# indygreg/python-zstandard

Measured on AMD Instinct MI355X. Metric: GB/s uncompressed throughput, batch decompress of 128 KiB level-3 frames (the decompress half of BASELINE.json's metric; the compress half on the same inputs is this line's 'compress' object), higher is better.
Workload: dtype u8

## Files before the change

### python-zstandard_amd/csrc/zhip_decode_pipeline.hpp

```cpp
#pragma once
#include "zhip_decode_kernel.hpp"

ZH_DEV void zp_pack_fse(ZdLDS& L, uint32_t* T, uint32_t llLog, uint32_t ofLog, uint32_t mlLog)
{
    const uint32_t lane = zh_lane();
    for (uint32_t u = lane; u < ZP_FSE_CELLS / 2; u += 64) {
        const uint32_t lg = u < 256 ? llLog : u < 512 ? mlLog : ofLog;
        const uint32_t local = (2 * u) & (u < 512 ? 511u : 255u);
        uint32_t pair = 0;
        for (uint32_t k = 0; k < 2; k++) {
            uint32_t cell = 0;
            if (local + k < (1u << lg)) {
                const uint32_t e = L.fse[2 * u + k];
                cell = ((e >> 19) << 10) | (((e & 1023) + (1u << lg)) >> ((e >> 10) & 15));
            }
            pair |= cell << (16 * k);
        }
        T[u] = pair;
    }
}

struct ZpHdr { uint32_t pos, blockMax, hasChecksum, skippable; uint64_t fcs; };
ZH_DEV int zp_frame_header(const ZhipPipeArgs& a, const uint8_t* src, uint32_t srcSize, ZpHdr& h)
{
// ... 867 lines not shown
#ifndef ZQ_FRAMES
#define ZQ_FRAMES 15
#endif
#define ZQ_ROWS 32
struct ZpSeqQLDS { uint32_t ring[(ZQ_ROWS + 1) * 16]; uint32_t llInfo[36]; uint32_t mlInfo[53]; uint32_t spare; uint8_t tab[ZQ_FRAMES * ZP_K2_STRIDE]; };

ZH_DEV uint32_t zq_field(const uint32_t* col, int32_t q, uint32_t width)
{
    const uint32_t* w = (const uint32_t*)((const uint8_t*)col + (zh_bfe((uint32_t)q, 5, 5) << 6));
    return zh_bfe(zh_alignbit(w[16], w[0], (uint32_t)q), 0, width);
}
ZH_DEV void zq_commit(uint32_t* col, int32_t off, const ZpVec16& v)
{
    const uint32_t r0 = ((uint32_t)off >> 2) & (ZQ_ROWS - 1);
    uint32_t* q = col + (r0 << 4);
    q[0] = v.a; q[16] = v.b; q[32] = v.c; q[48] = v.d;
    if (r0 == 0) col[ZQ_ROWS << 4] = v.a;
}
ZH_DEV ZpVec16 zq_fetch(const uint8_t* p0, int32_t off) { return *(const ZpVec16*)(p0 + (uint32_t)(off < 0 ? 0 : off)); }

#ifndef ZQ_FENCES
#define ZQ_FENCES 1
#endif
#if ZQ_FENCES >= 1
#define ZQ_F1() ZH_SCHED_FENCE()
#else
#define ZQ_F1() do { } while (0)
#endif
#if ZQ_FENCES >= 2
#define ZQ_F2() ZH_SCHED_FENCE()
#else
#define ZQ_F2() do { } while (0)
#endif
template <bool MB>
ZH_DEVFN void zp_seqq_body(const ZhipPipeArgs& a, ZpSeqQLDS& L)
{
    const uint32_t lane = zh_lane(), role = lane & 3, slot = lane >> 2;
    if (lane < 36) L.llInfo[lane] = zc_llBase[lane] | ((uint32_t)zc_llBits[lane] << 24);
    if (lane < 53) L.mlInfo[lane] = zc_mlBase[lane] | ((uint32_t)zc_mlBits[lane] << 24);
    if (lane == 0) L.spare = 512;
    zh_sync();
    const bool isOF = role == 0, isSpare = role == 3;
    const uint32_t* const info = role == 1 ? L.mlInfo : L.llInfo;
    const uint32_t tabOff = role == 0 ? ZP_FSE_OF : role == 1 ? ZP_FSE_ML : ZP_FSE_LL;
    const uint32_t total = a.counters[1];
    const uint32_t nGroups = (total + ZQ_FRAMES - 1) / ZQ_FRAMES;
    for (;;) {
        const uint32_t g = zh_first(zh_atomic_add(a.counters + 3, lane == 0 ? 1u : 0u));
        if (g >= nGroups) break;
        const uint32_t k = g * ZQ_FRAMES + slot;
        const bool active = slot < ZQ_FRAMES && k < total;
        const uint32_t i = active ? a.order[k] : 0xFFFFFFFFu;
        const uint32_t logs0 = active ? a.meta[i].logs : 0u;
        zh_sync();
        for (uint32_t j = 0; j < ZQ_FRAMES; j++) {
            const uint32_t fj = zh_shfl(i, 4 * j);
            if (fj == 0xFFFFFFFFu) break;
            const bool sharedT = (zh_shfl(logs0, 4 * j) & ZP_LOGS_SHARED) != 0;
            const uint32_t* src = sharedT ? (const uint32_t*)a.dictTables->fseK2 : (const uint32_t*)(a.fseTables + (size_t)fj * ZP_FSE_CELLS);
            uint32_t* dstw = (uint32_t*)(L.tab + (size_t)j * ZP_K2_STRIDE);
            uint32_t r[ZP_FSE_CELLS / 128];
#pragma unroll
            for (uint32_t q = 0; q < ZP_FSE_CELLS / 128; q++) r[q] = src[lane + 64 * q];
#pragma unroll
            for (uint32_t q = 0; q < ZP_FSE_CELLS / 128; q++) dstw[lane + 64 * q] = r[q];
        }
        uint32_t* const col = L.ring + (active ? slot : 0u);
        const bool idle = isSpare || !active;
        const uint16_t* const Tm = idle ? (const uint16_t*)&L.spare : (const uint16_t*)(L.tab + (size_t)slot * ZP_K2_STRIDE) + tabOff;
        ZdMeta* const m = a.meta + (active ? i : 0u);
        const uint32_t fi = active ? (MB ? a.itemFrame[i] : i) : 0u;
        const uint32_t f = a.first + fi;
        uint32_t nbSeq = 0, logs = 0;
        int32_t pos = 0, pb = -(1 << 30), fin = 0;
        const uint8_t* p0 = nullptr;
        bool ok = active;
        ZpVec16 v0, v1; v0.a = v0.b = v0.c = v0.d = 0; v1 = v0;
// ... 3 lines not shown
            const uint8_t* p = src + m->seqOff; const uint8_t* end = src + m->seqEnd;
            const uint32_t size = (uint32_t)(end - p);
            logs = m->logs;
            const uint32_t lastB = size ? p[size - 1] : 0u;
            if (lastB == 0) ok = false;
            else {
                nbSeq = m->nbSeq;
                const uint32_t mis = (uint32_t)((uintptr_t)p & 15);
                p0 = p - mis; fin = (int32_t)(8 * mis);
                const int32_t topByte = (int32_t)(mis + size) - 1;
                tb = topByte & ~15;
                v0 = zq_fetch(p0, tb - 16 * (int32_t)role); v1 = zq_fetch(p0, tb - 16 * (int32_t)(role + 4));
                pb = tb - 128;
                pos = 8 * topByte + zh_highbit32(lastB);
            }
        }
        if (ok) { zq_commit(col, tb - 16 * (int32_t)role, v0); zq_commit(col, tb - 16 * (int32_t)(role + 4), v1); }
        zh_sync();
        const uint32_t llLog = logs & 255, ofLog = (logs >> 8) & 255, mlLog = (logs >> 16) & 255;
        const uint32_t myLog = idle ? 9u : role == 0 ? ofLog : role == 1 ? mlLog : llLog;
        const uint32_t kk = 31 - myLog, size = 1u << myLog;
        const uint16_t* const Tb = Tm - size;
        uint32_t state;
        {   const uint32_t initOff = role == 0 ? llLog : role == 1 ? llLog + ofLog : 0u;
            state = idle ? size : size + zq_field(col, pos - (int32_t)(initOff + myLog), myLog);
            pos -= (int32_t)(llLog + ofLog + mlLog); }
        const uint32_t nTrips = zh_first(zh_wave_max(nbSeq)) + 5;
        uint32_t rep0 = 1, rep1 = 4, rep2 = 8;
        if (a.dictEntropy) { rep0 = a.dictEntropy->rep[0]; rep1 = a.dictEntropy->rep[1]; rep2 = a.dictEntropy->rep[2]; }
        if (MB && active && a.frameRecs[fi].firstItem != i) { rep0 = ZP_SYM_REP(0); rep1 = ZP_SYM_REP(1); rep2 = ZP_SYM_REP(2); }
        uint32_t fin0 = rep0, fin1 = rep1, fin2 = rep2;
        rep0 = zh_opaque(rep0); rep1 = zh_opaque(rep1); rep2 = zh_opaque(rep2);
        ZpVec16* outp;
        {
            const uint32_t per = ((nTrips - 5 + 3) & ~3u) + 8;
            const uint32_t nAct = (uint32_t)zh_popc64(zh_ballot(active)) >> 2;
            const uint32_t need16 = per * nAct / 2;
            const uint32_t room16 = zh_first(zh_atomic_add(a.counters + 7, lane == 0 ? need16 : 0u));
            const uint32_t room = room16 * 2;
            if ((uint64_t)room16 + need16 + a.counters[8] > a.arenaBudget16) {
                if (active && isOF) { m->path = 2; if (!MB) { const uint32_t q = zh_atomic_add(a.fallbackCount, 1u); a.fallbackList[q] = f; } }
                zh_sync();
                continue;
            }
            const uint32_t start = room + slot * per + 4;
            if (active && isOF) a.bases[2 * (size_t)i] = start;
            outp = (ZpVec16*)(a.seqArena + (isOF && active ? (size_t)start - 4 : (size_t)room + per - 4));
        }
        const uint32_t outStep = isOF && active ? 2u : 0u;
        uint32_t g1lo = 0, g1hi = 0, g2lo = 0, g2hi = 0, g3lo = 0, g3hi = 0;
        ZpVec16 w0, w1; w0.a = w0.b = w0.c = w0.d = 0; w1 = w0;
        int32_t boff = ZP_NOBLK, posEnd = pos; ZpVec16 blk = v0;
        uint32_t pe0 = 0, pe1 = 0, pqE = 0, pbits = 0, pbase = 1;
        for (uint32_t n0 = 0; n0 < nTrips; n0 += 4) {
            zh_sync();
            if (boff != ZP_NOBLK) { zq_commit(col, boff, blk); boff = ZP_NOBLK; }
            {
                const int32_t t = pb + 128 - (((pos >> 5) << 2) + 4);
                if ((int32_t)(role * 16) <= t) { boff = pb - 16 * (int32_t)role; blk = zq_fetch(p0, boff); }
                int32_t cnt = (t >> 4) + 1; cnt = cnt < 0 ? 0 : cnt > 4 ? 4 : cnt;
                pb -= 16 * cnt; }
#pragma unroll
            for (uint32_t u = 0; u < 4; u++) {
                const uint32_t n = n0 + u;
                const uint32_t cell = Tb[state];
                ZQ_F1();
                const uint32_t val = pbase + zh_bfe(zh_alignbit(pe1, pe0, pqE), 0, pbits);
                const uint32_t mlv = zh_quad<1>(val), llv = zh_quad<2>(val);
                const uint32_t idx = val - 1 + (llv == 0);
                const uint32_t vm3 = val - 3;
                const uint32_t newOff = vm3 < ZP_OF_LIMIT ? vm3 : ZP_OF_LIMIT;
                const uint32_t c3 = val > 3 ? newOff : rep0 - 1;
                uint32_t offset = idx == 2 ? rep2 : c3; offset = idx == 1 ? rep1 : offset; offset = idx == 0 ? rep0 : offset;
                ZQ_F2();
                const uint32_t sym = cell >> 10, x = cell & 1023;
                const uint32_t inf = info[sym];
                const uint32_t nb = (uint32_t)__builtin_clz(x) - kk;
                ZQ_F2();
                rep2 = idx <= 1 ? rep2 : rep1; rep1 = idx == 0 ? rep1 : rep0; rep0 = offset;
                if (MB) {
                    const bool wasLast = n == nbSeq;
                    fin0 = wasLast ? rep0 : fin0; fin1 = wasLast ? rep1 : fin1; fin2 = wasLast ? rep2 : fin2;
                }
                {   const uint32_t plo = llv | (mlv << 17), phi = (mlv >> 15) | (offset << 3);
                    if (u == 0) {
                        w0.a = g1lo; w0.b = g1hi; w0.c = g2lo; w0.d = g2hi; w1.a = g3lo; w1.b = g3hi; w1.c = plo; w1.d = phi;
#if defined(ZQ_DIAG_NOSTORE)
                        outp += outStep;
#elif defined(ZQ_NT_STORE)
                        {   typedef uint32_t zq_v4 __attribute__((ext_vector_type(4)));
                            zq_v4 t0 = { w0.a, w0.b, w0.c, w0.d }, t1 = { w1.a, w1.b, w1.c, w1.d };
                            __builtin_nontemporal_store(t0, (zq_v4*)outp); __builtin_nontemporal_store(t1, (zq_v4*)(outp + 1)); outp += outStep; }
#else
                        outp[0] = w0; outp[1] = w1; outp += outStep;
#endif
                    } else if (u == 1) { g1lo = plo; g1hi = phi; } else if (u == 2) { g2lo = plo; g2hi = phi; } else { g3lo = plo; g3hi = phi; } }
                ZQ_F2();
                const uint32_t bits = isOF ? sym : inf >> 24;
                const uint32_t P = zh_quad_add<0xCF>(zh_quad_add<0xD3>(bits, bits), bits);
                const uint32_t R = zh_quad_add<0xFE>(zh_quad_add<0xF9>(nb, nb), nb);
                const uint32_t totE = zh_quad<2>(P), totN = zh_quad<0>(R);
                const int32_t pE = pos - (int32_t)totE;
                const int32_t qS = pE - (int32_t)R, qE = pos - (int32_t)P;
                const uint32_t* const wS = (const uint32_t*)((const uint8_t*)col + (zh_bfe((uint32_t)qS, 5, 5) << 6));
                const uint32_t* const wE = (const uint32_t*)((const uint8_t*)col + (zh_bfe((uint32_t)qE, 5, 5) << 6));
                const uint32_t s0 = wS[0], s1 = wS[16];
                pe0 = wE[0]; pe1 = wE[16];
                ZQ_F2();
                pqE = (uint32_t)qE; pbits = bits;
                posEnd = n + 1 == nbSeq ? pE : posEnd;
                pos = pE - (int32_t)totN;
                pbase = isOF ? 1u << (sym & 31) : inf & 0xFFFFFFu;
                ZQ_F2();
                state = (x << nb) + zh_bfe(zh_alignbit(s1, s0, (uint32_t)qS), 0, nb);
            }
            ZH_KEEP4(w0.a, w0.b, w0.c, w0.d); ZH_KEEP4(w1.a, w1.b, w1.c, w1.d);
        }
        if (active && isOF) {
            const int err = !ok ? ZE_CORRUPTION : posEnd != fin ? ZE_CORRUPTION : 0;
            if (err) { m->status = err; m->path = 0; if (!MB) { a.status[f] = err; a.outSizes[f] = 0; } }
            if (MB) { uint32_t* r = a.itemReps + 4 * (size_t)i; r[0] = fin0; r[1] = fin1; r[2] = fin2; }
        }
        zh_sync();
    }
}

#ifndef ZP_ASM_BYTES
#define ZP_ASM_BYTES ZD_ASM_BYTES
#endif
struct ZpExecLDS {
    uint8_t asmb[ZP_ASM_BYTES + 64]; uint16_t mBeg[64]; uint16_t mEnd[64]; uint32_t misc[8];
#if defined(ZP_K3_DIAG_FLOOR) && defined(ZP_FLOOR_LDSPAD)
    uint8_t floorPad[ZP_FLOOR_LDSPAD];
#endif
    uint16_t uEnd[64], uLit[64], dstL[64], dstM[64], lenL[64], lenM[64]; uint32_t srcL[64], srcM[64];
};

ZH_DEV void zp_ld32_lds(const uint8_t* q, uint32_t len, uint64_t r[4])
{
    r[0] = zh_ld64(q); r[1] = zh_ld64(q + 8); r[2] = zh_ld64(q + 16);
    r[3] = zh_ld64(q + (len >= 8 ? len - 8 : 0u));
}

#ifndef ZP_LIT_SHORT
#define ZP_LIT_SHORT 16
#endif
#ifndef ZP_FAR_SHORT
#define ZP_FAR_SHORT 16
#endif
#ifndef ZP_K3_NT
#define ZP_K3_NT 0
#endif
#if ZP_K3_NT & 1
#define ZP_SEQ_LD(p) zh_ldq_nt(p)
#define ZP_LIT_LD64(p) zh_ld64_nt(p)
#else
#define ZP_SEQ_LD(p) (*(p))
#define ZP_LIT_LD64(p) zh_ld64(p)
#endif
#if ZP_K3_NT & 2
#define ZP_FAR_LD64(p) zh_ld64_nt(p)
#else
#define ZP_FAR_LD64(p) zh_ld64(p)
#endif
#define ZD_TP(P, i) do { if (PROF) ZD_T(P, i); } while (0)
ZH_DEV uint32_t zp_sym_resolve(uint32_t v, uint32_t R0, uint32_t R1, uint32_t R2)
{
    if (v <= ZP_OF_LIMIT) return v;
    if (v > ZP_SYM_TOP) return 0xFFFFFFFFu;
    const uint32_t k = (v - (ZP_OF_LIMIT + 1)) >> 23;
    const uint32_t d = ZP_SYM_REP(k) - v;
    const uint32_t r = k == 0 ? R0 : k == 1 ? R1 : R2;
    return r > d ? r - d : 0xFFFFFFFFu;
}

#define ZP_BSYNC() zh_sync()
#ifndef ZP_HIST_KEEP
#define ZP_HIST_KEEP ((ZP_ASM_BYTES * 5u / 16u) & ~15u)
#define ZP_HIST_SLIDE (2u * ZP_HIST_KEEP + 16u)
#endif
static_assert((ZP_HIST_SLIDE >= 2 * ZP_HIST_KEEP + 16 || ZP_HIST_KEEP == 0) && ZP_HIST_KEEP % 16 == 0 && ZP_HIST_SLIDE < ZP_ASM_BYTES, "the slide's source and destination must not overlap");
template <bool DICT, bool PROF, bool MB>
ZH_DEVFN int zp_exec_block(const ZhipPipeArgs& a, ZpExecLDS& L, const ZdMeta& m, uint32_t t, const uint8_t* src, uint8_t* dst, uint32_t cap, uint64_t cap64,
                           uint32_t blockMax, uint32_t& opRef, uint32_t R0, uint32_t R1, uint32_t R2, ZdProf& P)
{
    const uint32_t lane = zh_lane();
    const uint64_t* seqs = a.seqArena + a.bases[2 * (size_t)t];
    const bool litRLE = m.litMode == 2;
    const uint32_t rleByte = m.litOff;
    const uint8_t* litPtr = m.litMode == 0 ? src + m.litOff : a.litArena + (size_t)a.bases[2 * (size_t)t + 1] * 16;
    const uint8_t* const dictEnd = DICT ? a.dictContent + a.dictContentSize : dst;
    const uint32_t dictSize = DICT ? a.dictContentSize : 0u;
    uint32_t hOff = 0;
    uint8_t* asmb = L.asmb;
    const uint32_t blockStart = MB ? opRef : 0u;
    uint32_t op = blockStart, lp = 0, done = 0;
    uint32_t carry = 0;
    const uint32_t nbSeq = m.nbSeq;
    uint64_t qNext = lane < nbSeq ? ZP_SEQ_LD(seqs + lane) : 0;
    const uint32_t lane0 = lane;
    while (done < nbSeq) {
        const uint32_t avail = nbSeq - done < 64 ? nbSeq - done : 64;
        uint32_t myLL = 0, myML = 0, myOF = 1;
        if (lane < avail) { const uint64_t q = qNext; myLL = ZP_SEQ_LL(q); myML = ZP_SEQ_ML(q); myOF = ZP_SEQ_OF(q); if (MB) myOF = zp_sym_resolve(myOF, R0, R1, R2); }
        if (MB && zh_ballot(lane < avail && myOF == ZP_OF_LIMIT)) return ZP_RC_FALLBACK;
        uint32_t incL = zh_scan_add(myLL), incT = zh_scan_add(myLL + myML);
        const uint64_t fits = zh_ballot(lane < avail && incT + carry <= ZP_ASM_BYTES - hOff);
        uint32_t cnt = (uint32_t)zh_popc64(fits);
        const bool big = cnt == 0;
        if (big) cnt = 1;
        qNext = done + cnt + lane < nbSeq ? ZP_SEQ_LD(seqs + done + cnt + lane) : 0;
        const bool act = lane < cnt;
        if (!act) { myLL = 0; myML = 0; myOF = 1; }
        const uint32_t totL = zh_bcast(incL, cnt - 1), totT = zh_bcast(incT, cnt - 1);
        if (lp + totL > m.litSize) return ZE_CORRUPTION;
        if ((uint64_t)op + totT > cap) return ZE_DST_TOO_SMALL;
        if (op + totT - blockStart > blockMax) return ZE_CORRUPTION;
        const uint32_t litStart = lp + incL - myLL;
        const uint32_t ob = op - carry;
        const uint32_t oRel = incT - (myLL + myML) + carry, mRel = oRel + myLL;
        if (zh_ballot(act && myOF - 1 >= ob + mRel + dictSize)) return ZE_CORRUPTION;
        if (big) {
            if (lane < carry) dst[ob + lane] = asmb[lane];
            carry = 0;
            zd_fence();
            const uint32_t bll = zh_bcast(myLL, 0), bml = zh_bcast(myML, 0), bof = zh_bcast(myOF, 0);
            if (litRLE) zd_fill_wave(dst + op, rleByte, bll); else zd_copy_wave(dst + op, litPtr + lp, bll);
            zd_fence();
            zd_match_wave(dst, dictEnd, op + bll, bof, bml);
            zd_fence();
            op += totT; lp += totL; done += 1;
            hOff = 0; asmb = L.asmb;
            continue;
        }
        ZD_TP(P, ZP_STAGE);
        const int32_t sAbs = (int32_t)(ob + mRel) - (int32_t)myOF;
        const bool hasM = act && myML > 0;
        const bool farM = hasM && sAbs + (int32_t)myML <= (int32_t)ob;
        uint32_t nearSkip = 0;
        {
            uint64_t rl[4], rm[4];
            const bool shortL = act && myLL > 0 && myLL <= ZP_LIT_SHORT;
            const bool arenaLit = m.litMode != 0;
            if (arenaLit && !litRLE) {
// ... 99 lines not shown
                            if (c == span) span += span;
                        }
                    }
                    pending = false;
                }
                uint64_t newDone = zh_ballot(ready);
                for (uint64_t lm = longReady; lm; lm &= lm - 1) {
                    const uint32_t pf = (uint32_t)zh_ctz64(lm);
                    const uint32_t Frel = zh_shfl(mRel, pf), fml = zh_shfl(myML, pf), fof = zh_shfl(myOF, pf);
                    const int32_t fs = (int32_t)(ob + Frel) - (int32_t)fof;
                    if (fof >= 64) {
                        for (uint32_t c = 0; c < fml; c += 64) {
                            const uint32_t j = c + lane;
                            if (j < fml) { const int32_t sp = fs + (int32_t)j; asmb[Frel + j] = sp >= (int32_t)(ob - hOff) ? asmb[sp - (int32_t)ob] : (DICT ? (uint8_t)zd_hist_byte(dst, dictEnd, sp) : dst[sp]); }
                            if (fof < fml) ZP_BSYNC();
                        }
                    } else {
                        uint32_t idx = lane % fof; const uint32_t adv = 64 % fof;
                        for (uint32_t j = lane; j < fml; j += 64) {
                            const int32_t sp = fs + (int32_t)idx;
                            asmb[Frel + j] = sp >= (int32_t)(ob - hOff) ? asmb[sp - (int32_t)ob] : (DICT ? (uint8_t)zd_hist_byte(dst, dictEnd, sp) : dst[sp]);
                            idx += adv; if (idx >= fof) idx -= fof;
                        }
                    }
                    if (lane == pf) pending = false;
                    newDone |= 1ull << pf;
                    if (lm & (lm - 1)) ZP_BSYNC();
                }
                doneMask |= newDone;
            }
            ZP_BSYNC();
        }
        ZD_TP(P, ZP_EXEC2);
        qNext = zh_opaque64(qNext);
        const uint32_t totB = totT + carry, whole = totB & ~15u;
        {
            uint8_t* out = dst + ob;
            const uint32_t j0 = lane * 16;
            if (j0 < whole) { const zh_v16 v = *(const zh_v16*)(asmb + j0); *(zh_v16*)(out + j0) = v; }
            if (whole > 1024) for (uint32_t j = j0 + 1024; j < whole; j += 1024) { const zh_v16 v = *(const zh_v16*)(asmb + zh_opaque(j)); *(zh_v16*)(out + j) = v; }
        }
        carry = totB - whole;
        hOff += whole;
        ZP_BSYNC();
        if (hOff > ZP_HIST_SLIDE) {
            const uint32_t s0 = hOff - ZP_HIST_KEEP, n = ZP_HIST_KEEP + carry;
            for (uint32_t j = lane * 16; j < n; j += 1024) { const zh_v16 v = *(const zh_v16*)(L.asmb + s0 + j); *(zh_v16*)(L.asmb + j) = v; }
            hOff = ZP_HIST_KEEP;
            ZP_BSYNC();
        }
        asmb = L.asmb + hOff;
        ZD_TP(P, ZP_FLUSH);
        op += totT; lp += totL; done += cnt;
    }
    if (lane < carry) dst[op - carry + lane] = asmb[lane];
    zd_fence();
    const uint32_t rest = m.litSize - lp;
    if ((uint64_t)op + rest > cap) return ZE_DST_TOO_SMALL;
    if (op + rest - blockStart > blockMax) return ZE_CORRUPTION;
    if (litRLE) zd_fill_wave(dst + op, rleByte, rest); else zd_copy_wave(dst + op, litPtr + lp, rest);
    op += rest;
    opRef = op;
    return 0;
}


ZH_DEVFN int zp_exec_frame_end(ZpExecLDS& L, const uint8_t* dst, uint32_t op, uint32_t fcsLo, uint32_t fcsHi, uint32_t hasChecksum, uint32_t checksum, uint32_t ckLater)
{
    const uint32_t lane = zh_lane();
    const uint64_t fcs = (uint64_t)fcsLo | ((uint64_t)fcsHi << 32);
    if (fcs != ~0ull && fcs != op) return ZE_CORRUPTION;
    if ((hasChecksum & 1) && !ckLater) {
        zd_fence();
        zh_sync();
        if (zh_opaque(lane) == 0) L.misc[0] = (uint32_t)ze_xxh64(dst, op);
        zh_sync();
        const uint32_t digest = zh_first(L.misc[0]);
        zh_sync();
        if (digest != checksum) return ZE_CHECKSUM_WRONG;
    }
    return 0;
}

#ifdef ZP_K3_DIAG_FLOOR
#include "../../tests/ubench/k3_floor_diag.hpp"
#endif
template <bool DICT, bool PROF>
ZH_DEVFN int zp_exec_frame(const ZhipPipeArgs& a, ZpExecLDS& L, uint32_t i, uint32_t* pProduced, ZdProf& P)
{
    const ZdMeta m = a.meta[i];
    const uint32_t f = a.first + i;
    const uint8_t* src = a.src + a.srcSegs[2 * (size_t)f];
    uint8_t* dst = a.dst + a.dstSegs[2 * (size_t)f];
    const uint64_t cap64 = a.dstSegs[2 * (size_t)f + 1];
    const uint32_t cap = cap64 > 0x7FFFFFFFull ? 0x7FFFFFFFu : (uint32_t)cap64;
    uint32_t op = 0;
#ifdef ZP_K3_DIAG_FLOOR
// ... 100 lines not shown
```

### python-zstandard_amd/csrc/zhip_format.hpp

```cpp
#pragma once
#include <stdint.h>

enum {
    ZE_OK = 0, ZE_GENERIC = 1, ZE_PREFIX_UNKNOWN = 10, ZE_FRAMEPARAM_UNSUPPORTED = 14, ZE_WINDOW_TOO_LARGE = 16,
    ZE_CORRUPTION = 20, ZE_CHECKSUM_WRONG = 22, ZE_LITERALS_HEADER_WRONG = 24, ZE_DICT_CORRUPTED = 30,
    ZE_DICT_WRONG = 32, ZE_PARAM_UNSUPPORTED = 40, ZE_PARAM_OUTOFBOUND = 42, ZE_TABLELOG_TOO_LARGE = 44, ZE_MAXSYMBOL_TOO_LARGE = 46,
    ZE_MAXSYMBOL_TOO_SMALL = 48, ZE_MEMORY = 64, ZE_DST_TOO_SMALL = 70, ZE_SRC_SIZE_WRONG = 72
};

#define ZF_MAGIC 0xFD2FB528u
#define ZF_MAGIC_SKIPPABLE 0x184D2A50u
#define ZF_DICT_MAGIC 0xEC30A437u
#define ZF_BLOCK_MAX (1u << 17)
#define ZF_MAXLL 35
#define ZF_MAXML 52
#define ZF_MAXOFF 31
#define ZF_LL_LOGMAX 9
#define ZF_ML_LOGMAX 9
#define ZF_OF_LOGMAX 8

#define ZHIP_LIT_STRIDE (ZF_BLOCK_MAX + 256)

struct ZhipDictEntropy {
    uint8_t  hufWeights[256];
// ... 125 lines not shown
    int32_t  strat, tlen;
    uint32_t contentSize, dictID;
    uint32_t rep[3];
    uint32_t hufRepeat, llRepeat, ofRepeat, mlRepeat;
    uint32_t hufMaxSym;
    uint8_t  hufBits[256];
    uint16_t hufCode[256];
    ZeCTab   tab[3];
};

struct ZdMeta {
    int32_t  status;
    uint32_t path;
    uint32_t seqOff;
    uint32_t seqEnd;
    uint32_t litSize;
    uint32_t litMode;
    uint32_t litOff;
    uint32_t nbSeq;
    uint32_t blockMax;
    uint32_t fcsLo, fcsHi;
    uint32_t produced;
    uint32_t hasChecksum, checksum;
    uint32_t logs;
    uint32_t pad;
};
#define ZP_SEQ_CAP 45056u
#define ZP_SEQ_FRONT 16u
#define ZP_SEQ_STRIDE ((size_t)ZP_SEQ_CAP * 8)
#define ZP_SEQ_LL(q) ((uint32_t)(q) & 0x1FFFFu)
#define ZP_SEQ_ML(q) ((uint32_t)((q) >> 17) & 0x3FFFFu)
#define ZP_SEQ_OF(q) ((uint32_t)((q) >> 35))
#define ZP_SEQ_OFBITS 29
#define ZP_LIT_STRIDE ((size_t)ZF_BLOCK_MAX + 256)
#define ZP_LIT_FRONT 256u
#define ZP_FSE_LL 0
#define ZP_FSE_ML 512
#define ZP_FSE_OF 1024
#define ZP_FSE_CELLS 1280
#define ZP_K2_STRIDE 2564
#define ZP_HUF_LOGMAX 11
#define ZP_HUF_CELLS (1u << ZP_HUF_LOGMAX)
#ifndef ZP_HUF_FRAMES
#define ZP_HUF_FRAMES 12
#endif
#define ZP_HUF_LS (ZP_HUF_FRAMES > 8 ? 6 : ZP_HUF_FRAMES > 4 ? 5 : 4)
#define ZP_LITBIN_SHIFT 9
#define ZP_BIN_SHIFT 7

#define ZP_CNT_BINS 16u
#define ZP_CNT_WORDS (16u + 512u)

struct ZpFrameRec {
    uint32_t firstItem, nItems;
    uint32_t path;
    uint32_t blockMax;
    uint32_t fcsLo, fcsHi;
    uint32_t hasChecksum, checksum;
};
#define ZP_OF_LIMIT 0x1E000000u
#define ZP_SYM_REP(k) (0x1E800000u + ((uint32_t)(k) << 23))
#define ZP_SYM_TOP ZP_SYM_REP(2)
#define ZP_MB_MAXBLOCKS 4096u
#define ZP_RC_FALLBACK 0x7FFF0002
struct alignas(16) ZpPre {
    uint8_t weights[256];
// ... 40 lines not shown
```

### python-zstandard_amd/csrc/zhip_lib.hip

```cpp
#include <atomic>
#include <chrono>
#include <hip/hip_runtime.h>
#include <stdio.h>
#include <time.h>
#include <stdlib.h>
#include <string.h>
#include <string>
#include <vector>
#include "../../include/zstd_hip.h"
#include "zhip_decode_pipeline.hpp"
#include "zhip_encode_kernel.hpp"
#include "zhip_cparams.hpp"

#define ZHIP_LDS_BYTES (160u * 1024u)
#ifndef ZHIP_E1LDS_PER_CU
#define ZHIP_E1LDS_PER_CU 4
#endif
static_assert(sizeof(ZpSeqQLDS) <= ZHIP_LDS_BYTES && sizeof(ZpHufKernelLDS) <= ZHIP_LDS_BYTES, "a workgroup's LDS must fit a CU");

ZH_GLOBAL __launch_bounds__(64, 2) void zhip_decode_frames_kernel(ZhipDecodeArgs a)
{
    __shared__ ZdLDS L;
    zd_kernel_body(a, L);
}
ZH_GLOBAL __launch_bounds__(64, 2) void zhip_decode_lit_kernel(ZhipPipeArgs a)
{
    __shared__ ZdLDS L;
    zp_lit_body(a, L);
}
ZH_GLOBAL __launch_bounds__(64) void zhip_decode_lit_lanes_kernel(ZhipPipeArgs a) { zp_lit_lanes_body(a); }
ZH_GLOBAL __launch_bounds__(64) void zhip_decode_check_kernel(ZhipPipeArgs a) { zp_check_body(a); }
ZH_GLOBAL __launch_bounds__(64) void zhip_decode_pre_kernel(ZhipPipeArgs a)
{
    __shared__ ZpPreLDS L;
    zp_pre_body(a, L);
}
ZH_GLOBAL __launch_bounds__(64) void zhip_decode_bin_kernel(ZhipPipeArgs a)
{
    __shared__ ZpBinLDS L;
    zp_bin_body(a, L);
}
ZH_GLOBAL __launch_bounds__(64) void zhip_decode_huf_kernel(ZhipPipeArgs a)
{
    __shared__ ZpHufKernelLDS L;
    zp_huf_body(a, L);
}
ZH_GLOBAL __launch_bounds__(64) void zhip_decode_seq_kernel(ZhipPipeArgs a)
{
    __shared__ ZpSeqQLDS L;
    zp_seqq_body<false>(a, L);
}
ZH_GLOBAL __launch_bounds__(64, 2) void zhip_decode_lit_mb_kernel(ZhipPipeArgs a)
{
    __shared__ ZdLDS L;
    zp_lit_mb_body(a, L);
}
ZH_GLOBAL __launch_bounds__(64) void zhip_decode_seq_mb_kernel(ZhipPipeArgs a)
{
    __shared__ ZpSeqQLDS L;
    zp_seqq_body<true>(a, L);
}
#ifndef ZP_K3_MINWAVES
#define ZP_K3_MINWAVES 6
#endif
ZH_GLOBAL __launch_bounds__(64, ZP_K3_MINWAVES) void zhip_decode_exec_kernel(ZhipPipeArgs a)
{
    __shared__ ZpExecLDS L;
    zp_exec_body<false, false>(a, L);
}
ZH_GLOBAL __launch_bounds__(64, 4) void zhip_decode_exec_prof_kernel(ZhipPipeArgs a)
{
    __shared__ ZpExecLDS L;
    zp_exec_body<false, true>(a, L);
}
#ifndef ZP_K3D_MINWAVES
#define ZP_K3D_MINWAVES 4
#endif
ZH_GLOBAL __launch_bounds__(64, ZP_K3D_MINWAVES) void zhip_decode_exec_dict_kernel(ZhipPipeArgs a)
{
    __shared__ ZpExecLDS L;
    zp_exec_body<true, false>(a, L);
}
ZH_GLOBAL __launch_bounds__(64, 4) void zhip_decode_exec_mb_kernel(ZhipPipeArgs a)
{
    __shared__ ZpExecLDS L;
    zp_exec_body<false, false, true>(a, L);
}
ZH_GLOBAL __launch_bounds__(64, 4) void zhip_decode_exec_mb_dict_kernel(ZhipPipeArgs a)
{
    __shared__ ZpExecLDS L;
    zp_exec_body<true, false, true>(a, L);
}
ZH_GLOBAL __launch_bounds__(64, 3) void zhip_encode_frames_kernel(ZhipEncodeArgs a)
// ... 531 lines not shown
                                            int32_t* d_status, void* streamv)
{
    if (!c) return ZHIP_ERR_UNSUPPORTED;
    if (n == 0) return 0;
    if (n > 0x7FFFFFFFu) { g_lastError = "too many frames in one launch"; return ZHIP_ERR_UNSUPPORTED; }
    hipStream_t stream = (hipStream_t)streamv;
    size_t maxBlocks = (size_t)c->numCU * (size_t)c->decBlocksPerCU;
    uint32_t grid = (uint32_t)(n < maxBlocks ? n : maxBlocks);
    if (c->scratch.reserve((size_t)grid * ZHIP_LIT_STRIDE)) return g_reserveRc;
    if (c->counter.reserve(64)) return g_reserveRc;
    HIP_TRY(hipMemsetAsync(c->counter.p, 0, 4, stream));
    const uint32_t* d_fallbackList = nullptr; const uint32_t* d_fallbackCount = nullptr;
    const bool usePipeline = true;
    if (usePipeline) {
        const size_t chunkMax = c->knob.dchunk; int slotMax = c->knob.nslot;
        const uint64_t sizeHint = c->dstMaxHint ? c->dstMaxHint : c->itemHint;
        if (!c->knob.nslotSet && sizeHint && sizeHint <= 16384 && slotMax < 3) slotMax = 3;
        const bool mb = sizeHint > ZF_BLOCK_MAX && sizeHint <= 0x7FFFFFFFull;
        const bool side = ZHIP_SIDE && !c->hostPipe && !(sizeHint && sizeHint <= 16384);
        if (side) slotMax = 1;
        const size_t perFrame = mb ? (size_t)(2 * ((sizeHint + ZF_BLOCK_MAX - 1) / ZF_BLOCK_MAX) + 2) : 1;
        const size_t slotsHint = mb ? c->dstSlotsHint : 0;
        const size_t chunkFrames = !mb ? chunkMax : slotsHint ? (size_t)((double)n * (double)(chunkMax / 2) / (double)slotsHint) + 1 : (chunkMax / perFrame ? chunkMax / perFrame : 1);
        const size_t chunk = n < chunkFrames ? n : chunkFrames;
        auto slotsFor = [&](size_t frames) {
            if (!mb) return frames;
            if (slotsHint) { const size_t want = 2 * (size_t)((double)frames * (double)slotsHint / (double)n + 1.0) + 64; return want < frames ? frames : want; }
            const size_t lo = frames * perFrame, hi = 2 * lo < chunkMax ? 2 * lo : chunkMax; return lo > hi ? lo : hi; };
        const size_t slots = slotsFor(chunk);
        if (slots > 0x7FFFFFFFu) { g_lastError = "frame too large for the block arenas"; return ZHIP_ERR_UNSUPPORTED; }
        const size_t nChunks = (n + chunk - 1) / chunk;
        const int nslot = (int)(nChunks < (size_t)slotMax ? nChunks : (size_t)slotMax);
        const size_t floorFrames = slots < 1024 ? slots : 1024;
        const size_t smallWorst = !mb && sizeHint && sizeHint < ZF_BLOCK_MAX ? 4 * (size_t)sizeHint + 1024 : (size_t)0;
        const size_t roomPerFrame = smallWorst && smallWorst < (160u << 10) ? smallWorst : (size_t)(160u << 10);
        size_t arenaBudget16 = slots * (roomPerFrame / 16);
        const size_t worstFrame = smallWorst ? smallWorst : (size_t)(ZP_SEQ_STRIDE + ZP_LIT_STRIDE);
        if (arenaBudget16 < floorFrames * (worstFrame / 16)) arenaBudget16 = floorFrames * (worstFrame / 16);
        if (arenaBudget16 > 0xFFFFFFF0u) arenaBudget16 = 0xFFFFFFF0u;
        const size_t arenaBytes = arenaBudget16 * 16 + 512;
        if (c->pipeBases.reserve(nslot * slots * 2 * sizeof(uint32_t))) return g_reserveRc;
        if (c->pipeMeta.reserve(nslot * slots * sizeof(ZdMeta)) || c->pipeLit.reserve(nslot * arenaBytes + ZP_LIT_FRONT) || c->pipeCounters.reserve((8 + (size_t)ZHIP_NSLOT * ZP_CNT_WORDS) * 4) || c->pipeFallback.reserve(n * 4 + 16) ||
            c->pipeFse.reserve(nslot * slots * ZP_FSE_CELLS * sizeof(uint16_t)) || c->pipeOrder.reserve(nslot * slots * sizeof(uint32_t)) ||
            c->pipeHuf.reserve(nslot * slots * ZP_HUF_CELLS * sizeof(uint16_t)) || c->pipeOrderLit.reserve(nslot * slots * sizeof(uint32_t))) return g_reserveRc;
        const bool pre = ZHIP_K0 && !mb && !c->dictHasEntropy && chunk >= c->knob.k0Min;
        if (pre && c->pipePre.reserve(nslot * slots * sizeof(ZpPre))) return g_reserveRc;
        if (mb && (c->pipeItemFrame.reserve(nslot * slots * sizeof(uint32_t)) || c->pipeItemReps.reserve(nslot * slots * 4 * sizeof(uint32_t)) ||
                   c->pipeFrameRecs.reserve(nslot * chunk * sizeof(ZpFrameRec)))) return g_reserveRc;
        for (int sidx = 0; sidx < nslot; sidx++) if (!c->slotStream[sidx]) HIP_TRY(hipStreamCreateWithFlags(&c->slotStream[sidx], hipStreamNonBlocking));
        HIP_TRY(hipMemsetAsync(c->pipeCounters.p, 0, (8 + (size_t)ZHIP_NSLOT * ZP_CNT_WORDS) * 4, stream));
        hipEvent_t evStart; HIP_TRY(hipEventCreateWithFlags(&evStart, hipEventDisableTiming));
        HIP_TRY(hipEventRecord(evStart, stream));
        for (int sidx = 0; sidx < nslot; sidx++) HIP_TRY(hipStreamWaitEvent(c->slotStream[sidx], evStart, 0));
        (void)hipEventDestroy(evStart);
        ZhipPipeArgs pa; memset(&pa, 0, sizeof pa);
        pa.src = (const uint8_t*)d_src; pa.srcSegs = (const uint64_t*)d_srcSegs; pa.dst = (uint8_t*)d_dst; pa.dstSegs = (const uint64_t*)d_dstSegs;
        pa.outSizes = d_outSizes; pa.status = d_status; pa.fallbackList = (uint32_t*)c->pipeFallback.p;
        pa.maxWindowSize = c->maxWindowSize; pa.magicless = c->dformat == ZHIP_FORMAT_ZSTD1_MAGICLESS;
        if (c->dictSize) {
            pa.dictID = c->dictID;
            pa.dictContent = (const uint8_t*)c->dictBlob.p + c->dictContentOffset;
            pa.dictContentSize = c->dictSize - c->dictContentOffset;
            pa.dictEntropy = c->dictHasEntropy ? (const ZhipDictEntropy*)c->dictEntropy.p : nullptr;
            pa.dictTables = c->dictHasEntropy ? (const ZhipDictTables*)c->dictTables.p : nullptr;
        }
        if (c->knob.prof) {
            if (!c->profPipe && (c->dictSize || mb))
                fprintf(stderr, "[zhip-prof] K3's phase timers exist in the dictionary-less single-block kernel only: with a dictionary or frames of several blocks they read zero\n");
            if (!c->profPipe) HIP_TRY(hipMalloc((void**)&c->profPipe, 32 * 8));
            HIP_TRY(hipMemsetAsync(c->profPipe, 0, 32 * 8, stream));
// ... 28 lines not shown
            if (c->knob.k3PerCU) g3m = (size_t)c->numCU * (size_t)c->knob.k3PerCU;
            if (c->knob.k1PerCU) g1m = (size_t)c->numCU * (size_t)c->knob.k1PerCU;
            const size_t w2 = (items + ZQ_FRAMES - 1) / ZQ_FRAMES, g2m = (size_t)c->numCU * (ZHIP_LDS_BYTES / sizeof(ZpSeqQLDS));
            pa.k1Lanes = !mb && c->dictHasEntropy ? 1u : 0u;
            pa.ckLater = 1;
            pa.pre = pre ? (ZpPre*)c->pipePre.p + (size_t)sidx * slots : nullptr;
            const size_t tasks1 = cnt;
            const uint32_t g1 = (uint32_t)(tasks1 < g1m ? tasks1 : g1m), g2 = (uint32_t)(w2 < g2m ? w2 : g2m), g3 = (uint32_t)(cnt < g3m ? cnt : g3m);
            const size_t wh = (items + ZP_HUF_FRAMES - 1) / ZP_HUF_FRAMES, ghm = (size_t)c->numCU * (ZHIP_LDS_BYTES / sizeof(ZpHufKernelLDS));
            const uint32_t gh = (uint32_t)(wh < ghm ? wh : ghm);
            const bool tm = c->timing;
            hipEvent_t ev[4] = {nullptr, nullptr, nullptr, nullptr}, evh = nullptr, evh2 = nullptr;
            if (tm) {
                for (int i = 0; i < 4; i++) HIP_TRY(hipEventCreate(&ev[i]));
                HIP_TRY(hipEventCreate(&evh)); HIP_TRY(hipEventCreate(&evh2));
                HIP_TRY(hipEventRecord(ev[0], ss));
            }
            if (mb) hipLaunchKernelGGL(zhip_decode_lit_mb_kernel, dim3(g1), dim3(64), 0, ss, pa);
            else {
                if (pa.pre) { const size_t w = (cnt + 63) / 64, gm = (size_t)c->numCU * 7; hipLaunchKernelGGL(zhip_decode_pre_kernel, dim3((uint32_t)(w < gm ? w : gm)), dim3(64), 0, ss, pa); }
                if (pa.k1Lanes) { const size_t w = (cnt + 63) / 64; hipLaunchKernelGGL(zhip_decode_lit_lanes_kernel, dim3((uint32_t)(w < g1m ? w : g1m)), dim3(64), 0, ss, pa); }
                hipLaunchKernelGGL(zhip_decode_lit_kernel, dim3(g1), dim3(64), 0, ss, pa);
            }
            hipLaunchKernelGGL(zhip_decode_bin_kernel, dim3(2 * (items < 4096 ? 1u : 64u)), dim3(64), 0, ss, pa);
            hipEvent_t evS0 = nullptr, evS1 = nullptr;
            if (side) {
                if (!c->sideStream[sidx]) HIP_TRY(hipStreamCreateWithFlags(&c->sideStream[sidx], hipStreamNonBlocking));
                hipStream_t sd = c->sideStream[sidx];
                hipEvent_t evBin, evSide; HIP_TRY(hipEventCreateWithFlags(&evBin, hipEventDisableTiming)); HIP_TRY(hipEventCreateWithFlags(&evSide, hipEventDisableTiming));
                if (tm) { HIP_TRY(hipEventRecord(evh, ss)); HIP_TRY(hipEventRecord(evh2, ss)); HIP_TRY(hipEventCreate(&evS0)); HIP_TRY(hipEventCreate(&evS1)); }
                HIP_TRY(hipEventRecord(evBin, ss));
                HIP_TRY(hipStreamWaitEvent(sd, evBin, 0));
                if (mb) hipLaunchKernelGGL(zhip_decode_seq_mb_kernel, dim3(g2), dim3(64), 0, ss, pa);
                else hipLaunchKernelGGL(zhip_decode_seq_kernel, dim3(g2), dim3(64), 0, ss, pa);
                if (tm) { HIP_TRY(hipEventRecord(ev[1], ss)); HIP_TRY(hipEventRecord(evS0, ss)); }
                hipLaunchKernelGGL(zhip_decode_huf_kernel, dim3(gh), dim3(64), 0, sd, pa);
                if (tm) HIP_TRY(hipEventRecord(evS1, sd));
                HIP_TRY(hipEventRecord(evSide, sd));
                HIP_TRY(hipStreamWaitEvent(ss, evSide, 0));
                (void)hipEventDestroy(evBin); (void)hipEventDestroy(evSide);
                if (tm) HIP_TRY(hipEventRecord(ev[2], ss));
            } else {
                if (tm) { HIP_TRY(hipEventRecord(evh, ss)); HIP_TRY(hipEventRecord(evh2, ss)); }
                hipLaunchKernelGGL(zhip_decode_huf_kernel, dim3(gh), dim3(64), 0, ss, pa);
                if (tm) HIP_TRY(hipEventRecord(ev[1], ss));
                if (mb) hipLaunchKernelGGL(zhip_decode_seq_mb_kernel, dim3(g2), dim3(64), 0, ss, pa);
                else hipLaunchKernelGGL(zhip_decode_seq_kernel, dim3(g2), dim3(64), 0, ss, pa);
                if (tm) HIP_TRY(hipEventRecord(ev[2], ss));
            }
            if (mb && pa.dictContent) hipLaunchKernelGGL(zhip_decode_exec_mb_dict_kernel, dim3(g3), dim3(64), 0, ss, pa);
            else if (mb) hipLaunchKernelGGL(zhip_decode_exec_mb_kernel, dim3(g3), dim3(64), 0, ss, pa);
            else if (pa.dictContent) hipLaunchKernelGGL(zhip_decode_exec_dict_kernel, dim3(g3), dim3(64), 0, ss, pa);
            else if (pa.prof) hipLaunchKernelGGL(zhip_decode_exec_prof_kernel, dim3(g3), dim3(64), 0, ss, pa);
            else hipLaunchKernelGGL(zhip_decode_exec_kernel, dim3(g3), dim3(64), 0, ss, pa);
            { const size_t w = (cnt + 63) / 64, gm = (size_t)c->numCU * 8; hipLaunchKernelGGL(zhip_decode_check_kernel, dim3((uint32_t)(w < gm ? w : gm)), dim3(64), 0, ss, pa); }
            if (tm) HIP_TRY(hipEventRecord(ev[3], ss));
            HIP_TRY(hipGetLastError());
            if (tm) {
                c->timer[2].pending.emplace_back(ev[0], evh);
                if (side) {
                    c->timer[3].pending.emplace_back(evh2, ev[1]);
                    c->timer[7].pending.emplace_back(evS0, evS1);
                } else {
                    c->timer[7].pending.emplace_back(evh2, ev[1]);
                    c->timer[3].shared.emplace_back(ev[1], ev[2]);
                }
                c->timer[9].shared.emplace_back(ev[0], ev[3]);
                c->timer[4].pending.emplace_back(ev[2], ev[3]);
            }
        }
        if (pa.prof) {
            HIP_TRY(hipDeviceSynchronize());
            unsigned long long h[32];
            HIP_TRY(hipMemcpy(h, pa.prof, sizeof h, hipMemcpyDeviceToHost));
            static const char* nm[10] = {"header", "huf-table", "huf-decode", "seq-header+fse", "K3 load+scan", "-", "K3 literal/far fetch", "K3 near rounds", "K3 flush", "tail"};
            for (int k = 0; k < 2; k++) {
                unsigned long long tot = 0; for (int q = 0; q < 10; q++) tot += h[16 * k + q];
                fprintf(stderr, "[zhip-prof] %s: %.0f wave-cycles per frame\n", k ? "K3" : "K1", (double)tot / (double)n);
                for (int q = 0; q < 10; q++) if (h[16 * k + q]) fprintf(stderr, "[zhip-prof]    %-22s %6.2f%% %10.0f cyc/frame\n", nm[q], 100.0 * h[16 * k + q] / (tot ? tot : 1), (double)h[16 * k + q] / (double)n);
// ... 976 lines not shown
```

Before: 394.5.

## Pack decoded sequences into 32-bit words with escape overflow records

```diff
diff --git a/profiles/seq_field_widths.py b/profiles/seq_field_widths.py
--- /dev/null
+++ b/profiles/seq_field_widths.py
@@ -0,0 +1,52 @@
+import ctypes as C
+import os
+import sys
+import numpy as np
+sys.path.insert(0, os.path.dirname(os.path.dirname(os.path.abspath(__file__))))
+from tests.corpus import Corpus
+from tests import reflib
+
+n = int(sys.argv[1]) if len(sys.argv) > 1 else 1024
+corpus = Corpus(mix="silesia")
+enc = reflib.RefZstd() if reflib.have_ref() else reflib.Oracle()
+L = C.CDLL(reflib.ORACLE_SO)
+L.zo_set_seq_trace.argtypes = [C.c_void_p, C.c_size_t]
+L.zo_seq_trace_count.restype = C.c_size_t
+L.zo_decompress_frame.restype = C.c_int64
+L.zo_decompress_frame.argtypes = [C.c_void_p, C.c_size_t, C.c_void_p, C.c_size_t, C.c_void_p, C.c_size_t, C.c_void_p]
+buf = np.zeros((1 << 16, 3), dtype=np.uint32)
+out = C.create_string_buffer(131072)
+raws = corpus.frame_list(0, n)
+seqs, csz = [], 0
+for r in raws:
+    f = enc.compress(r)
+    csz += len(f)
+    L.zo_set_seq_trace(buf.ctypes.data, buf.shape[0])
+    assert L.zo_decompress_frame(out, 131072, f, len(f), None, 0, None) == len(r)
+    seqs.append(buf[: L.zo_seq_trace_count()].copy())
+L.zo_set_seq_trace(None, 0)
+S = np.concatenate([a for a in seqs if len(a)])
+ll, ml, of = S[:, 0].astype(np.int64), S[:, 1].astype(np.int64), S[:, 2].astype(np.int64)
+ns = np.array([len(a) for a in seqs])
+print("encoder: %s" % ("reference libzstd" if reflib.have_ref() else "oracle"))
+print("frames %d  ratio %.3f  sequences %d  per frame: mean %.0f p50 %d p90 %d max %d" % (n, n * 131072 / csz, len(S), ns.mean(), np.median(ns), np.percentile(ns, 90), ns.max()))
+print("max ll %d  max ml %d  max offset %d (a single-block 128 KiB frame cannot reach past its start: < 2^17)" % (ll.max(), ml.max(), of.max()))
+
+
+def hist(name, v, edges):
+    h = np.histogram(v, bins=edges)[0] / len(v)
+    print("%-3s %s" % (name, "  ".join("<%d:%.4f" % (e, x) for e, x in zip(edges[1:], h))))
+
+
+hist("ll", ll, [0, 1, 2, 4, 8, 16, 32, 64, 128, 256, 512, 1024, 1 << 20])
+hist("ml", ml, [0, 4, 8, 16, 32, 64, 128, 256, 512, 1024, 2048, 1 << 20])
+hist("of", of, [0, 16, 256, 4096, 16384, 32768, 65536, 131072, 1 << 32])
+print("ll bits + ml bits | fit | escaped ll / ml | escapes per frame mean / max | 64-sequence runs with an escape | 4-sequence store groups with an ll / ml escape")
+for a in range(4, 12):
+    b = 15 - a
+    el, em = ll >= (1 << a) - 1, ml >= (1 << b) - 1
+    per = [int(((x[:, 0] >= (1 << a) - 1) | (x[:, 1] >= (1 << b) - 1)).sum()) if len(x) else 0 for x in seqs]
+    nb, ng = len(S) // 64 * 64, len(S) // 4 * 4
+    print("  %2d + %2d   %.4f   %.4f / %.4f   %.1f / %d   %.3f   %.4f / %.4f" % (
+        a, b, (~(el | em)).mean(), el.mean(), em.mean(), np.mean(per), max(per), (el | em)[:nb].reshape(-1, 64).any(axis=1).mean(),
+        el[:ng].reshape(-1, 4).any(axis=1).mean(), em[:ng].reshape(-1, 4).any(axis=1).mean()))
diff --git a/python-zstandard_amd/csrc/zhip_decode_pipeline.hpp b/python-zstandard_amd/csrc/zhip_decode_pipeline.hpp
--- a/python-zstandard_amd/csrc/zhip_decode_pipeline.hpp
+++ b/python-zstandard_amd/csrc/zhip_decode_pipeline.hpp
@@ -923,9 +923,10 @@
 #else
 #define ZQ_F2() do { } while (0)
 #endif
-template <bool MB>
-ZH_DEVFN void zp_seqq_body(const ZhipPipeArgs& a, ZpSeqQLDS& L)
-{
+template <bool MB, bool W32>
+ZH_DEVFN void zp_seqq_form(const ZhipPipeArgs& a, ZpSeqQLDS& L)
+{
+    static_assert(!(MB && W32), "the several-block mode keeps the 8-byte form");
     const uint32_t lane = zh_lane(), role = lane & 3, slot = lane >> 2;
     if (lane < 36) L.llInfo[lane] = zc_llBase[lane] | ((uint32_t)zc_llBits[lane] << 24);
     if (lane < 53) L.mlInfo[lane] = zc_mlBase[lane] | ((uint32_t)zc_mlBits[lane] << 24);
@@ -934,6 +935,8 @@
     const bool isOF = role == 0, isSpare = role == 3;
     const uint32_t* const info = role == 1 ? L.mlInfo : L.llInfo;
     const uint32_t tabOff = role == 0 ? ZP_FSE_OF : role == 1 ? ZP_FSE_ML : ZP_FSE_LL;
+    const uint32_t wSat = role == 1 ? ZP_W_MLSAT : role == 2 ? ZP_W_LLSAT : 0xFFFFFFFFu;
+    const uint32_t wEsc = role == 0 ? 0u : wSat;
     const uint32_t total = a.counters[1];
     const uint32_t nGroups = (total + ZQ_FRAMES - 1) / ZQ_FRAMES;
     for (;;) {
@@ -1003,10 +1006,11 @@
         uint32_t fin0 = rep0, fin1 = rep1, fin2 = rep2;
         rep0 = zh_opaque(rep0); rep1 = zh_opaque(rep1); rep2 = zh_opaque(rep2);
         ZpVec16* outp;
+        ZpVec16* park = nullptr;
         {
             const uint32_t per = ((nTrips - 5 + 3) & ~3u) + 8;
             const uint32_t nAct = (uint32_t)zh_popc64(zh_ballot(active)) >> 2;
-            const uint32_t need16 = per * nAct / 2;
+            const uint32_t need16 = W32 ? 3 * per / 4 * nAct : per * nAct / 2;
             const uint32_t room16 = zh_first(zh_atomic_add(a.counters + 7, lane == 0 ? need16 : 0u));
             const uint32_t room = room16 * 2;
             if ((uint64_t)room16 + need16 + a.counters[8] > a.arenaBudget16) {
@@ -1014,11 +1018,19 @@
                 zh_sync();
                 continue;
             }
+            if (W32) {
+                ZpVec16* const base = (ZpVec16*)a.litArena + room16;
+                const uint32_t fr16 = slot * (3 * per / 4);
+                if (active && isOF) { a.bases[2 * (size_t)i] = room16 + fr16 + 1; m->pad = per; }
+                park = base + (per / 4 - 1);
+                outp = !active || isSpare ? park : isOF ? base + fr16 : base + fr16 + (per / 4 - 2) + (role == 1 ? 1u : 0u);
+            } else {
             const uint32_t start = room + slot * per + 4;
             if (active && isOF) a.bases[2 * (size_t)i] = start;
             outp = (ZpVec16*)(a.seqArena + (isOF && active ? (size_t)start - 4 : (size_t)room + per - 4));
-        }
-        const uint32_t outStep = isOF && active ? 2u : 0u;
+            }
+        }
+        const uint32_t outStep = W32 ? (!active || isSpare ? 0u : isOF ? 1u : 2u) : isOF && active ? 2u : 0u;
         uint32_t g1lo = 0, g1hi = 0, g2lo = 0, g2hi = 0, g3lo = 0, g3hi = 0;
         ZpVec16 w0, w1; w0.a = w0.b = w0.c = w0.d = 0; w1 = w0;
         int32_t boff = ZP_NOBLK, posEnd = pos; ZpVec16 blk = v0;
@@ -1037,10 +1049,12 @@
                 const uint32_t cell = Tb[state];
                 ZQ_F1();
                 const uint32_t val = pbase + zh_bfe(zh_alignbit(pe1, pe0, pqE), 0, pbits);
-                const uint32_t mlv = zh_quad<1>(val), llv = zh_quad<2>(val);
+                const uint32_t sv = W32 ? (val < wSat ? val : wSat) : val;
+                const uint32_t mlv = zh_quad<1>(sv), llv = zh_quad<2>(sv);
                 const uint32_t idx = val - 1 + (llv == 0);
                 const uint32_t vm3 = val - 3;
-                const uint32_t newOff = vm3 < ZP_OF_LIMIT ? vm3 : ZP_OF_LIMIT;
+                const uint32_t ofLim = W32 ? ZP_W_OFSAT : ZP_OF_LIMIT;
+                const uint32_t newOff = vm3 < ofLim ? vm3 : ofLim;
                 const uint32_t c3 = val > 3 ? newOff : rep0 - 1;
                 uint32_t offset = idx == 2 ? rep2 : c3; offset = idx == 1 ? rep1 : offset; offset = idx == 0 ? rep0 : offset;
                 ZQ_F2();
@@ -1053,6 +1067,14 @@
                     const bool wasLast = n == nbSeq;
                     fin0 = wasLast ? rep0 : fin0; fin1 = wasLast ? rep1 : fin1; fin2 = wasLast ? rep2 : fin2;
                 }
+                if (W32) {
+                    const uint32_t d = isOF ? llv | (mlv << ZP_W_LLBITS) | (offset << 15) : val;
+                    if (u == 0) {
+                        w0.a = g1lo; w0.b = g2lo; w0.c = g3lo; w0.d = d;
+                        const uint32_t m12 = g1lo > g2lo ? g1lo : g2lo, m3d = g3lo > d ? g3lo : d, mx = m12 > m3d ? m12 : m3d;
+                        *(mx >= wEsc ? outp : park) = w0; outp += outStep;
+                    } else if (u == 1) g1lo = d; else if (u == 2) g2lo = d; else g3lo = d;
+                } else
                 {   const uint32_t plo = llv | (mlv << 17), phi = (mlv >> 15) | (offset << 3);
                     if (u == 0) {
                         w0.a = g1lo; w0.b = g1hi; w0.c = g2lo; w0.d = g2hi; w1.a = g3lo; w1.b = g3hi; w1.c = plo; w1.d = phi;
@@ -1095,6 +1117,13 @@
         zh_sync();
     }
 }
+template <bool MB>
+ZH_DEVFN void zp_seqq_body(const ZhipPipeArgs& a, ZpSeqQLDS& L)
+{
+    if constexpr (MB) zp_seqq_form<true, false>(a, L);
+    else if (a.dictContent) zp_seqq_form<false, false>(a, L);
+    else zp_seqq_form<false, true>(a, L);
+}
 
 #ifndef ZP_ASM_BYTES
 #define ZP_ASM_BYTES ZD_ASM_BYTES
@@ -1151,12 +1180,19 @@
 #define ZP_HIST_SLIDE (2u * ZP_HIST_KEEP + 16u)
 #endif
 static_assert((ZP_HIST_SLIDE >= 2 * ZP_HIST_KEEP + 16 || ZP_HIST_KEEP == 0) && ZP_HIST_KEEP % 16 == 0 && ZP_HIST_SLIDE < ZP_ASM_BYTES, "the slide's source and destination must not overlap");
+template <bool W32> struct ZpSeqWord { typedef uint64_t T; };
+template <> struct ZpSeqWord<true> { typedef uint32_t T; };
 template <bool DICT, bool PROF, bool MB>
 ZH_DEVFN int zp_exec_block(const ZhipPipeArgs& a, ZpExecLDS& L, const ZdMeta& m, uint32_t t, const uint8_t* src, uint8_t* dst, uint32_t cap, uint64_t cap64,
                            uint32_t blockMax, uint32_t& opRef, uint32_t R0, uint32_t R1, uint32_t R2, ZdProf& P)
 {
     const uint32_t lane = zh_lane();
+    constexpr bool W32 = !DICT && !MB;
+    typedef typename ZpSeqWord<W32>::T SeqT;
     const uint64_t* seqs = a.seqArena + a.bases[2 * (size_t)t];
+    const uint32_t* const words = (const uint32_t*)(a.litArena + (size_t)a.bases[2 * (size_t)t] * 16);
+    const uint32_t* const ovf = words + m.pad - 4;
+#define ZP_SEQ_GET(k) (W32 ? (SeqT)words[k] : (SeqT)ZP_SEQ_LD(seqs + (k)))
     const bool litRLE = m.litMode == 2;
     const uint32_t rleByte = m.litOff;
     const uint8_t* litPtr = m.litMode == 0 ? src + m.litOff : a.litArena + (size_t)a.bases[2 * (size_t)t + 1] * 16;
@@ -1168,11 +1204,20 @@
     uint32_t op = blockStart, lp = 0, done = 0;
     uint32_t carry = 0;
     const uint32_t nbSeq = m.nbSeq;
-    uint64_t qNext = lane < nbSeq ? ZP_SEQ_LD(seqs + lane) : 0;
+    SeqT qNext = lane < nbSeq ? ZP_SEQ_GET(lane) : 0;
     const uint32_t lane0 = lane;
     while (done < nbSeq) {
         const uint32_t avail = nbSeq - done < 64 ? nbSeq - done : 64;
         uint32_t myLL = 0, myML = 0, myOF = 1;
+        if (W32) {
+            if (lane < avail) { const uint32_t q = (uint32_t)qNext; myLL = ZP_W_LL(q); myML = ZP_W_ML(q); myOF = ZP_W_OF(q); }
+            const bool escL = lane < avail && myLL == ZP_W_LLSAT, escM = lane < avail && myML == ZP_W_MLSAT;
+            if (zh_ballot(escL || escM)) {
+                const uint32_t n = done + lane, o = 8 * (n >> 2) + (n & 3);
+                if (escL) myLL = ovf[o];
+                if (escM) myML = ovf[o + 4];
+            }
+        } else
         if (lane < avail) { const uint64_t q = qNext; myLL = ZP_SEQ_LL(q); myML = ZP_SEQ_ML(q); myOF = ZP_SEQ_OF(q); if (MB) myOF = zp_sym_resolve(myOF, R0, R1, R2); }
         if (MB && zh_ballot(lane < avail && myOF == ZP_OF_LIMIT)) return ZP_RC_FALLBACK;
         uint32_t incL = zh_scan_add(myLL), incT = zh_scan_add(myLL + myML);
@@ -1180,7 +1225,7 @@
         uint32_t cnt = (uint32_t)zh_popc64(fits);
         const bool big = cnt == 0;
         if (big) cnt = 1;
-        qNext = done + cnt + lane < nbSeq ? ZP_SEQ_LD(seqs + done + cnt + lane) : 0;
+        qNext = done + cnt + lane < nbSeq ? ZP_SEQ_GET(done + cnt + lane) : 0;
         const bool act = lane < cnt;
         if (!act) { myLL = 0; myML = 0; myOF = 1; }
         const uint32_t totL = zh_bcast(incL, cnt - 1), totT = zh_bcast(incT, cnt - 1);
@@ -1346,7 +1391,7 @@
             ZP_BSYNC();
         }
         ZD_TP(P, ZP_EXEC2);
-        qNext = zh_opaque64(qNext);
+        if (W32) qNext = (SeqT)zh_opaque((uint32_t)qNext); else qNext = (SeqT)zh_opaque64((uint64_t)qNext);
         const uint32_t totB = totT + carry, whole = totB & ~15u;
         {
             uint8_t* out = dst + ob;
@@ -1377,6 +1422,7 @@
     opRef = op;
     return 0;
 }
+#undef ZP_SEQ_GET
 
 
 ZH_DEVFN int zp_exec_frame_end(ZpExecLDS& L, const uint8_t* dst, uint32_t op, uint32_t fcsLo, uint32_t fcsHi, uint32_t hasChecksum, uint32_t checksum, uint32_t ckLater)
diff --git a/python-zstandard_amd/csrc/zhip_format.hpp b/python-zstandard_amd/csrc/zhip_format.hpp
--- a/python-zstandard_amd/csrc/zhip_format.hpp
+++ b/python-zstandard_amd/csrc/zhip_format.hpp
@@ -181,6 +181,13 @@
 #define ZP_SEQ_ML(q) ((uint32_t)((q) >> 17) & 0x3FFFFu)
 #define ZP_SEQ_OF(q) ((uint32_t)((q) >> 35))
 #define ZP_SEQ_OFBITS 29
+#define ZP_W_LLBITS 8
+#define ZP_W_LLSAT ((1u << ZP_W_LLBITS) - 1u)
+#define ZP_W_MLSAT ((1u << (15 - ZP_W_LLBITS)) - 1u)
+#define ZP_W_OFSAT 0x1FFFFu
+#define ZP_W_LL(w) ((w) & ZP_W_LLSAT)
+#define ZP_W_ML(w) (((w) >> ZP_W_LLBITS) & ZP_W_MLSAT)
+#define ZP_W_OF(w) ((w) >> 15)
 #define ZP_LIT_STRIDE ((size_t)ZF_BLOCK_MAX + 256)
 #define ZP_LIT_FRONT 256u
 #define ZP_FSE_LL 0
diff --git a/python-zstandard_amd/csrc/zhip_lib.hip b/python-zstandard_amd/csrc/zhip_lib.hip
--- a/python-zstandard_amd/csrc/zhip_lib.hip
+++ b/python-zstandard_amd/csrc/zhip_lib.hip
@@ -48,7 +48,12 @@
 ZH_GLOBAL __launch_bounds__(64) void zhip_decode_seq_kernel(ZhipPipeArgs a)
 {
     __shared__ ZpSeqQLDS L;
-    zp_seqq_body<false>(a, L);
+    zp_seqq_form<false, true>(a, L);
+}
+ZH_GLOBAL __launch_bounds__(64) void zhip_decode_seq_dict_kernel(ZhipPipeArgs a)
+{
+    __shared__ ZpSeqQLDS L;
+    zp_seqq_form<false, false>(a, L);
 }
 ZH_GLOBAL __launch_bounds__(64, 2) void zhip_decode_lit_mb_kernel(ZhipPipeArgs a)
 {
@@ -58,7 +63,7 @@
 ZH_GLOBAL __launch_bounds__(64) void zhip_decode_seq_mb_kernel(ZhipPipeArgs a)
 {
     __shared__ ZpSeqQLDS L;
-    zp_seqq_body<true>(a, L);
+    zp_seqq_form<true, false>(a, L);
 }
 #ifndef ZP_K3_MINWAVES
 #define ZP_K3_MINWAVES 6
@@ -656,10 +661,12 @@
         const size_t nChunks = (n + chunk - 1) / chunk;
         const int nslot = (int)(nChunks < (size_t)slotMax ? nChunks : (size_t)slotMax);
         const size_t floorFrames = slots < 1024 ? slots : 1024;
-        const size_t smallWorst = !mb && sizeHint && sizeHint < ZF_BLOCK_MAX ? 4 * (size_t)sizeHint + 1024 : (size_t)0;
-        const size_t roomPerFrame = smallWorst && smallWorst < (160u << 10) ? smallWorst : (size_t)(160u << 10);
+        const bool w32 = !mb && !c->dictSize;
+        const size_t smallWorst = !mb && sizeHint && sizeHint < ZF_BLOCK_MAX ? (w32 ? 5 : 4) * (size_t)sizeHint + 1024 : (size_t)0;
+        const size_t roomAvg = (size_t)(w32 ? 192u : 160u) << 10;
+        const size_t roomPerFrame = smallWorst && smallWorst < roomAvg ? smallWorst : roomAvg;
         size_t arenaBudget16 = slots * (roomPerFrame / 16);
-        const size_t worstFrame = smallWorst ? smallWorst : (size_t)(ZP_SEQ_STRIDE + ZP_LIT_STRIDE);
+        const size_t worstFrame = smallWorst ? smallWorst : (size_t)(ZP_SEQ_STRIDE * (w32 ? 3 : 2) / 2 + ZP_LIT_STRIDE);
         if (arenaBudget16 < floorFrames * (worstFrame / 16)) arenaBudget16 = floorFrames * (worstFrame / 16);
         if (arenaBudget16 > 0xFFFFFFF0u) arenaBudget16 = 0xFFFFFFF0u;
         const size_t arenaBytes = arenaBudget16 * 16 + 512;
@@ -754,6 +761,7 @@
                 HIP_TRY(hipEventRecord(evBin, ss));
                 HIP_TRY(hipStreamWaitEvent(sd, evBin, 0));
                 if (mb) hipLaunchKernelGGL(zhip_decode_seq_mb_kernel, dim3(g2), dim3(64), 0, ss, pa);
+                else if (pa.dictContent) hipLaunchKernelGGL(zhip_decode_seq_dict_kernel, dim3(g2), dim3(64), 0, ss, pa);
                 else hipLaunchKernelGGL(zhip_decode_seq_kernel, dim3(g2), dim3(64), 0, ss, pa);
                 if (tm) { HIP_TRY(hipEventRecord(ev[1], ss)); HIP_TRY(hipEventRecord(evS0, ss)); }
                 hipLaunchKernelGGL(zhip_decode_huf_kernel, dim3(gh), dim3(64), 0, sd, pa);
@@ -767,6 +775,7 @@
                 hipLaunchKernelGGL(zhip_decode_huf_kernel, dim3(gh), dim3(64), 0, ss, pa);
                 if (tm) HIP_TRY(hipEventRecord(ev[1], ss));
                 if (mb) hipLaunchKernelGGL(zhip_decode_seq_mb_kernel, dim3(g2), dim3(64), 0, ss, pa);
+                else if (pa.dictContent) hipLaunchKernelGGL(zhip_decode_seq_dict_kernel, dim3(g2), dim3(64), 0, ss, pa);
                 else hipLaunchKernelGGL(zhip_decode_seq_kernel, dim3(g2), dim3(64), 0, ss, pa);
                 if (tm) HIP_TRY(hipEventRecord(ev[2], ss));
             }
```

After: 396.6 (median of 6 runs). About the same (+0.5%).
